# chaitjo/efficient-gnns

Hardware: NVIDIA H100
Metric: edges aggregated/s (fwd+bwd), 3-layer GCN student + logit-KD, ARXIV-shape (higher is better)
Workload: dtype f32

## Files before the change

### efficient-gnns_b200/csrc/gemm_tf32x3.cu

```cuda
#include <cuda.h>

#include "common.cuh"
#include "tc_common.cuh"

namespace b200gnn {
namespace gemm {
using namespace tc;

constexpr int BM = 128, BK = 32;
constexpr int THREADS = 384;
constexpr int CONSUMER_WARPS = 8;
constexpr int TILE_BYTES = BM * BK * 4;
constexpr int WG_TILE_BYTES = TILE_BYTES / 2;
constexpr int BAR_BYTES = 256;
constexpr int EPI_BYTES = CONSUMER_WARPS * 16 * 32 * 4;
constexpr int STAT_MAX_N = 256;
constexpr int STAT_BYTES = CONSUMER_WARPS * 2 * STAT_MAX_N * 4;
constexpr int XY_ROWS = 16;
constexpr int XY_SLOT_BYTES = 2 * XY_ROWS * 32 * 4;
constexpr int XY_BYTES = CONSUMER_WARPS * 2 * XY_SLOT_BYTES;
constexpr int XY_BAR_OFF = 128;
constexpr int BNBWD_TMA_MAX_K = 128;

template <int BN_T, int NSTAGE, int EXTRA = 0>
struct Cfg {
  static constexpr int BN = BN_T, STAGES = NSTAGE;
  static constexpr int B_TILE_BYTES = BN_T * BK * 4;
  static constexpr int STAGE_BYTES = 2 * TILE_BYTES + 2 * B_TILE_BYTES;
  static constexpr int ACC = BN_T / 2;
  static constexpr int SMEM_BYTES = NSTAGE * STAGE_BYTES + BAR_BYTES + EPI_BYTES + STAT_BYTES + EXTRA + 1024;
  static_assert(B_TILE_BYTES % 1024 == 0 && (BN_T == 128 || BN_T == 48), "tile shape (wgmma wrappers: N = 128, 48)");
  static_assert(2 * NSTAGE * 8 <= XY_BAR_OFF, "barrier block");
  static_assert(SMEM_BYTES <= 232448, "shared memory");
};

__device__ __forceinline__ void mma(float (&d)[64], uint64_t a, uint64_t b, uint32_t s) { wgmma_tf32_n128(d, a, b, s); }
__device__ __forceinline__ void mma(float (&d)[24], uint64_t a, uint64_t b, uint32_t s) { wgmma_tf32_n48(d, a, b, s); }

__device__ __forceinline__ int stg(int r, int c4) { return r * 32 + ((c4 ^ (r & 7)) << 2); }

struct Params {
  float* C;
  const float* bias;
  int64_t ldc;
  int32_t M, N, K;
  int32_t accumulate;
  float* Cp[16];
  int32_t n_peer, kc;
  int64_t row_off;
  int32_t bcast;
  int32_t stat_mode;
  float* stat_partial;
  const float* bn_x;
  const float* bn_y;
  const float* bn_mean;
  const float* bn_invstd;
  float inv_keep;
};

__device__ __forceinline__ void load_bn_chunk(const Params& p, int m0, int col, int q, int lane, float4 (&x)[4], float4 (&y)[4]) {
  if (col + 32 > p.N) return;
  const int sub = lane >> 3, cq = (lane & 7) * 4;
#pragma unroll
  for (int it = 0; it < 4; ++it) {
    const int grow = m0 + q * 16 + it * 4 + sub;
    if (grow < p.M) {
      const size_t o = (size_t)grow * p.ldc + col + cq;
      x[it] = __ldg(reinterpret_cast<const float4*>(p.bn_x + o));
      y[it] = __ldg(reinterpret_cast<const float4*>(p.bn_y + o));
    }
// ... 13 lines not shown
  uint64_t* bars = reinterpret_cast<uint64_t*>(smem + STAGES * STAGE_BYTES);
  uint64_t* full = bars;
  uint64_t* empty = bars + STAGES;
  float* epi_smem = reinterpret_cast<float*>(smem + STAGES * STAGE_BYTES + BAR_BYTES);
  float* stat_smem = reinterpret_cast<float*>(smem + STAGES * STAGE_BYTES + BAR_BYTES + EPI_BYTES);
  uint8_t* xy_smem = smem + STAGES * STAGE_BYTES + BAR_BYTES + EPI_BYTES + STAT_BYTES;
  uint64_t* xy_full = reinterpret_cast<uint64_t*>(smem + STAGES * STAGE_BYTES + XY_BAR_OFF);

  const int warp = threadIdx.x >> 5, lane = threadIdx.x & 31;

  if (threadIdx.x == 0) {
    for (int s = 0; s < STAGES; ++s) { mbar_init(&full[s], 1); mbar_init(&empty[s], 256); }
    if (XYTMA)
      for (int i = 0; i < 2 * CONSUMER_WARPS; ++i) mbar_init(&xy_full[i], 1);
    asm volatile("fence.mbarrier_init.release.cluster;" ::: "memory");
  }
  __syncthreads();

  const int num_m = (p.M + BM - 1) / BM, num_n = (p.N + BN - 1) / BN;
  const int num_tiles = num_m * num_n;
  const int num_kb = (p.K + BK - 1) / BK;

  if (warp < 4) {
    regs_dec<40>();
    if (threadIdx.x == 0) {
      int s = 0; uint32_t ph = 0;
      for (int tile = blockIdx.x; tile < num_tiles; tile += gridDim.x) {
        const int m0 = (tile / num_n) * BM, n0 = (tile % num_n) * BN;
        for (int kb = 0; kb < num_kb; ++kb) {
          mbar_wait(&empty[s], ph ^ 1);
          uint8_t* st = smem + s * STAGE_BYTES;
          mbar_expect_tx(&full[s], TILE_BYTES + 2 * B_TILE_BYTES);
          tma_load_2d(&tmA, &full[s], st, kb * BK, m0);
          tma_load_2d(&tmBhi, &full[s], st + 2 * TILE_BYTES, kb * BK, n0);
          tma_load_2d(&tmBlo, &full[s], st + 2 * TILE_BYTES + B_TILE_BYTES, kb * BK, n0);
          if (++s == STAGES) { s = 0; ph ^= 1; }
        }
      }
    }
    return;
  }
  regs_inc<232>();

  const int cw = (warp >> 2) - 1;
  const int t = threadIdx.x & 127;
  const int q = warp - 4;
  const bool vec_ok = PEER ? true : ((p.ldc % 4 == 0) && ((reinterpret_cast<uintptr_t>(p.C) & 15) == 0));
  float* stat = stat_smem + q * (2 * STAT_MAX_N);
  if (STAT) {
    for (int i = lane; i < 2 * p.N; i += 32) stat[i] = 0.f;
    __syncwarp();
  }
  constexpr int NCHUNK = (BN + 31) / 32;
  uint8_t* xy = xy_smem + q * (2 * XY_SLOT_BYTES);
  uint64_t* xyb = xy_full + q * 2;
  int n_mine = 0;
  if (XYTMA) {
    for (int tt = blockIdx.x; tt < num_tiles; tt += gridDim.x) n_mine += NCHUNK;
    if (lane == 0)
      for (int g = 0; g < 2 && g < n_mine; ++g) {
        const int tt = blockIdx.x + (g / NCHUNK) * gridDim.x, cc = g % NCHUNK;
        mbar_expect_tx(&xyb[g], XY_SLOT_BYTES);
        tma_load_2d(&tmX, &xyb[g], xy + g * XY_SLOT_BYTES, (tt % num_n) * BN + cc * 32, (tt / num_n) * BM + q * XY_ROWS);
        tma_load_2d(&tmY, &xyb[g], xy + g * XY_SLOT_BYTES + XY_SLOT_BYTES / 2, (tt % num_n) * BN + cc * 32,
                    (tt / num_n) * BM + q * XY_ROWS);
      }
  }
  float acc[ACC], sum[ACC];
  int s = 0; uint32_t ph = 0;
  int g_chunk = 0;
  for (int tile = blockIdx.x; tile < num_tiles; tile += gridDim.x) {
    const int m0 = (tile / num_n) * BM, n0 = (tile % num_n) * BN;
#pragma unroll
    for (int i = 0; i < ACC; ++i) sum[i] = 0.f;
    int prev = 0;
    for (int kb = 0; kb < num_kb; ++kb) {
      mbar_wait(&full[s], ph);
      uint8_t* st = smem + s * STAGE_BYTES;
      {
        uint4* hi = reinterpret_cast<uint4*>(st + cw * WG_TILE_BYTES);
        uint4* lo = reinterpret_cast<uint4*>(st + TILE_BYTES + cw * WG_TILE_BYTES);
#pragma unroll
        for (int i = 0; i < WG_TILE_BYTES / 16 / 128; ++i) {
          const int o = i * 128 + t;
          const uint4 v = hi[o];
          uint4 h, l;
          split4(v, h, l);
          hi[o] = h;
          lo[o] = l;
        }
      }
      asm volatile("fence.proxy.async.shared::cta;" ::: "memory");
      named_sync(1 + cw, 128);
      if (kb > 0) {
        wgmma_wait<0>();
        acc_fence(acc);
#pragma unroll
        for (int i = 0; i < ACC; ++i) sum[i] += acc[i];
        mbar_arrive(&empty[prev]);
      }
      wgmma_fence();
      const uint32_t sa = smem_u32(st);
#pragma unroll
      for (int k = 0; k < BK / 8; ++k) {
        const uint32_t koff = k * 32;
        const uint64_t a_hi = make_desc_k128(sa + cw * WG_TILE_BYTES + koff);
        const uint64_t a_lo = make_desc_k128(sa + TILE_BYTES + cw * WG_TILE_BYTES + koff);
        const uint64_t b_hi = make_desc_k128(sa + 2 * TILE_BYTES + koff);
        const uint64_t b_lo = make_desc_k128(sa + 2 * TILE_BYTES + B_TILE_BYTES + koff);
        mma(acc, a_lo, b_hi, k != 0);
        mma(acc, a_hi, b_lo, 1);
      }
#pragma unroll
      for (int k = 0; k < BK / 8; ++k) {
        const uint32_t koff = k * 32;
        mma(acc, make_desc_k128(sa + cw * WG_TILE_BYTES + koff), make_desc_k128(sa + 2 * TILE_BYTES + koff), 1);
      }
      wgmma_commit();
      prev = s;
      if (++s == STAGES) { s = 0; ph ^= 1; }
    }
    wgmma_wait<0>();
    acc_fence(acc);
#pragma unroll
    for (int i = 0; i < ACC; ++i) sum[i] += acc[i];
    mbar_arrive(&empty[prev]);

    float* tile_s = epi_smem + q * (16 * 32);
#pragma unroll
    for (int c = 0; c < NCHUNK; ++c, ++g_chunk) {
      const int col0 = n0 + c * 32;
      float4 xr[4], yr[4];
      if (STAT == 2) load_bn_chunk(p, m0, col0, q, lane, xr, yr);
#pragma unroll
      for (int jj = 0; jj < 4; ++jj) {
        const int j = c * 4 + jj;
        if (j * 8 < BN) {
          const int r0 = lane >> 2, cc = jj * 8 + 2 * (lane & 3);
          *reinterpret_cast<float2*>(tile_s + stg(r0, cc >> 2) + (cc & 3)) = make_float2(sum[4 * j], sum[4 * j + 1]);
          *reinterpret_cast<float2*>(tile_s + stg(r0 + 8, cc >> 2) + (cc & 3)) = make_float2(sum[4 * j + 2], sum[4 * j + 3]);
        }
      }
      __syncwarp();
      if (vec_ok && col0 + 32 <= p.N) {
        const float* xs = reinterpret_cast<const float*>(xy + (g_chunk & 1) * XY_SLOT_BYTES);
        const float* ys = xs + XY_ROWS * 32;
        if (XYTMA) mbar_wait(&xyb[g_chunk & 1], (uint32_t)((g_chunk >> 1) & 1));
        const int sub = lane >> 3, cq = (lane & 7) * 4;
        float4 b4 = make_float4(0.f, 0.f, 0.f, 0.f);
        if (p.bias) b4 = make_float4(__ldg(p.bias + col0 + cq), __ldg(p.bias + col0 + cq + 1), __ldg(p.bias + col0 + cq + 2),
                                     __ldg(p.bias + col0 + cq + 3));
        float4 s4 = make_float4(0.f, 0.f, 0.f, 0.f), q4 = s4, mu4 = s4, is4 = s4;
        if (BNB) {
// ... 136 lines not shown
}
}

using namespace b200gnn;

extern "C" int b200gnn_split_tf32_f32(const float* W, int64_t rows, int64_t cols, int transpose, float* hi, float* lo,
                                      void* stream) {
  if (!W || !hi || !lo || rows <= 0 || cols <= 0) return B200GNN_ERR_BAD_ARG;
  const int64_t n = rows * cols;
  int grid = (int)((n + 255) / 256);
  if (grid > 132 * 8) grid = 132 * 8;
  gemm::split_tf32_kernel<<<grid, 256, 0, (cudaStream_t)stream>>>(W, rows, cols, transpose, hi, lo);
  return check_launch();
}

static int g_bnbwd_variant = 0;
extern "C" void b200gnn_gemm_set_bnbwd_variant(int v) { g_bnbwd_variant = v; }

static int gemm_dispatch(const float* A, int64_t lda, const float* B_hi, const float* B_lo, int64_t ldb, float* C, int64_t ldc,
                         int64_t M, int64_t N, int64_t K, const float* bias, int accumulate, void* stream,
                         const gemm::Params* st = nullptr) {
  if (!A || !B_hi || !B_lo || !C || M <= 0 || N <= 0 || K <= 0 || lda < K || ldb < K || ldc < N ||
      M >= INT32_MAX || N >= INT32_MAX || K >= INT32_MAX)
    return B200GNN_ERR_BAD_ARG;
  if (lda % 4 || ldb % 4 || !aligned_to(A, 16) || !aligned_to(B_hi, 16) || !aligned_to(B_lo, 16))
    return B200GNN_ERR_UNSUPPORTED;
  gemm::Params p{};
  p.C = C; p.bias = bias; p.ldc = ldc; p.M = (int32_t)M; p.N = (int32_t)N; p.K = (int32_t)K; p.accumulate = accumulate ? 1 : 0;
  p.n_peer = 0; p.kc = 0; p.row_off = 0; p.bcast = 0;
  if (st) {
    if (N % 32 || N > gemm::STAT_MAX_N || N <= 48 || ldc % 4 || !aligned_to(C, 16) || !st->stat_partial) return B200GNN_ERR_UNSUPPORTED;
    p.stat_mode = st->stat_mode; p.stat_partial = st->stat_partial; p.bn_x = st->bn_x; p.bn_y = st->bn_y;
    p.bn_mean = st->bn_mean; p.bn_invstd = st->bn_invstd; p.inv_keep = st->inv_keep;
    if (p.stat_mode == 1) return gemm::launch<gemm::Cfg<128, 3>, 1>(A, lda, B_hi, B_lo, ldb, p, (cudaStream_t)stream);
    if (N % 128 == 0 && (g_bnbwd_variant == 1 || (g_bnbwd_variant == 0 && K < gemm::BNBWD_TMA_MAX_K)))
      return gemm::launch<gemm::Cfg<128, 2, gemm::XY_BYTES>, 3>(A, lda, B_hi, B_lo, ldb, p, (cudaStream_t)stream);
    return gemm::launch<gemm::Cfg<128, 3>, 2>(A, lda, B_hi, B_lo, ldb, p, (cudaStream_t)stream);
  }
  if (N <= 48) return gemm::launch<gemm::Cfg<48, 4>>(A, lda, B_hi, B_lo, ldb, p, (cudaStream_t)stream);
  return gemm::launch<gemm::Cfg<128, 3>>(A, lda, B_hi, B_lo, ldb, p, (cudaStream_t)stream);
}

extern "C" int64_t b200gnn_gemm_stat_slots(int64_t M, int64_t N) {
  if (M <= 0 || N <= 0) return B200GNN_ERR_BAD_ARG;
  int dev = 0, sms = 132;
  cudaGetDevice(&dev);
  cudaDeviceGetAttribute(&sms, cudaDevAttrMultiProcessorCount, dev);
  const int64_t tiles = ((M + gemm::BM - 1) / gemm::BM) * ((N + 127) / 128);
  return gemm::CONSUMER_WARPS * (tiles < sms ? tiles : sms);
}

extern "C" int b200gnn_gemm_tf32x3_stats_f32(const float* A, int64_t lda, const float* B_hi, const float* B_lo, int64_t ldb,
                                             float* C, int64_t ldc, int64_t M, int64_t N, int64_t K, const float* bias,
                                             int accumulate, float* partial, int64_t slots, void* stream) {
  if (!partial || slots < b200gnn_gemm_stat_slots(M, N) || (accumulate && bias)) return B200GNN_ERR_BAD_ARG;
  gemm::Params st{};
  st.stat_mode = 1; st.stat_partial = partial;
  return gemm_dispatch(A, lda, B_hi, B_lo, ldb, C, ldc, M, N, K, bias, accumulate, stream, &st);
}

extern "C" int b200gnn_gemm_tf32x3_bnbwd_f32(const float* A, int64_t lda, const float* B_hi, const float* B_lo, int64_t ldb,
                                             float* C, int64_t ldc, int64_t M, int64_t N, int64_t K, int accumulate,
                                             const float* Xout, const float* Y, const float* mean, const float* invstd, float p_drop,
                                             float* partial, int64_t slots, void* stream) {
  if (!partial || !Xout || !Y || !mean || !invstd || p_drop < 0.f || p_drop >= 1.f || slots < b200gnn_gemm_stat_slots(M, N))
    return B200GNN_ERR_BAD_ARG;
  if (!aligned_to(Xout, 16) || !aligned_to(Y, 16) || !aligned_to(mean, 16) || !aligned_to(invstd, 16)) return B200GNN_ERR_UNSUPPORTED;
  gemm::Params st{};
  st.stat_mode = 2; st.stat_partial = partial; st.bn_x = Xout; st.bn_y = Y; st.bn_mean = mean; st.bn_invstd = invstd;
  st.inv_keep = p_drop > 0.f ? 1.f / (1.f - p_drop) : 1.f;
  return gemm_dispatch(A, lda, B_hi, B_lo, ldb, C, ldc, M, N, K, nullptr, accumulate, stream, &st);
}

extern "C" int b200gnn_gemm_tf32x3_f32(const float* A, int64_t lda, const float* B_hi, const float* B_lo, int64_t ldb,
                                       float* C, int64_t ldc, int64_t M, int64_t N, int64_t K, const float* bias,
                                       void* stream) {
  return gemm_dispatch(A, lda, B_hi, B_lo, ldb, C, ldc, M, N, K, bias, 0, stream);
}

extern "C" int b200gnn_gemm_tf32x3_acc_f32(const float* A, int64_t lda, const float* B_hi, const float* B_lo, int64_t ldb,
                                           float* C, int64_t ldc, int64_t M, int64_t N, int64_t K, void* stream) {
  return gemm_dispatch(A, lda, B_hi, B_lo, ldb, C, ldc, M, N, K, nullptr, 1, stream);
}

extern "C" int b200gnn_gemm_tf32x3_scatter_f32(const float* A, int64_t lda, const float* B_hi, const float* B_lo, int64_t ldb,
                                               float* const* C_ptrs, int32_t world, int64_t row_off, int64_t M, int64_t N, int64_t K,
                                               const float* bias, void* stream) {
  if (!A || !B_hi || !B_lo || !C_ptrs || world <= 0 || world > 16 || M <= 0 || N <= 0 || K <= 0 || lda < K || ldb < K || row_off < 0 ||
      M >= INT32_MAX || N >= INT32_MAX || K >= INT32_MAX)
    return B200GNN_ERR_BAD_ARG;
  if (N % world || (N / world) % 32 || N <= 48) return B200GNN_ERR_UNSUPPORTED;
  if (lda % 4 || ldb % 4 || !aligned_to(A, 16) || !aligned_to(B_hi, 16) || !aligned_to(B_lo, 16)) return B200GNN_ERR_UNSUPPORTED;
  gemm::Params p{};
  p.C = nullptr; p.bias = bias; p.ldc = N; p.M = (int32_t)M; p.N = (int32_t)N; p.K = (int32_t)K; p.accumulate = 0;
  p.n_peer = world; p.kc = (int32_t)(N / world); p.row_off = row_off; p.bcast = 0;
  for (int q = 0; q < world; ++q) {
    if (!C_ptrs[q] || !aligned_to(C_ptrs[q], 16)) return B200GNN_ERR_BAD_ARG;
    p.Cp[q] = C_ptrs[q];
  }
  return gemm::launch<gemm::Cfg<128, 3>, 0, true>(A, lda, B_hi, B_lo, ldb, p, (cudaStream_t)stream);
}

extern "C" int b200gnn_gemm_tf32x3_bcast_f32(const float* A, int64_t lda, const float* B_hi, const float* B_lo, int64_t ldb,
                                             float* const* C_ptrs, int32_t world, int64_t row_off, int64_t ldc, int64_t M, int64_t N,
                                             int64_t K, const float* bias, void* stream) {
  if (!A || !B_hi || !B_lo || !C_ptrs || world <= 0 || world > 16 || M <= 0 || N <= 0 || K <= 0 || lda < K || ldb < K || ldc < N ||
      row_off < 0 || M >= INT32_MAX || N >= INT32_MAX || K >= INT32_MAX)
    return B200GNN_ERR_BAD_ARG;
  if (lda % 4 || ldb % 4 || ldc % 4 || !aligned_to(A, 16) || !aligned_to(B_hi, 16) || !aligned_to(B_lo, 16)) return B200GNN_ERR_UNSUPPORTED;
  gemm::Params p{};
  p.C = C_ptrs[0]; p.bias = bias; p.ldc = ldc; p.M = (int32_t)M; p.N = (int32_t)N; p.K = (int32_t)K; p.accumulate = 0;
  p.n_peer = world; p.kc = (int32_t)N; p.row_off = row_off; p.bcast = 1;
  for (int q = 0; q < world; ++q) {
    if (!C_ptrs[q] || !aligned_to(C_ptrs[q], 16)) return B200GNN_ERR_BAD_ARG;
    p.Cp[q] = C_ptrs[q];
  }
  if (N <= 48) return gemm::launch<gemm::Cfg<48, 4>, 0, true>(A, lda, B_hi, B_lo, ldb, p, (cudaStream_t)stream);
  return gemm::launch<gemm::Cfg<128, 3>, 0, true>(A, lda, B_hi, B_lo, ldb, p, (cudaStream_t)stream);
}
```

### efficient-gnns_b200/csrc/gemm_wgrad_tf32x3.cu

```cuda
#include "common.cuh"
#include "tc_common.cuh"

namespace b200gnn {
namespace wgrad {
using namespace tc;

constexpr int BKN = 32;
constexpr int TM = 128, TN = 128;
constexpr int THREADS = 384;
constexpr int STAGES = 3;
constexpr int RAW_BYTES = BKN * (TM + TN) * 4;
constexpr int OP_BYTES = 128 * BKN * 4;
constexpr int T_BYTES = 4 * OP_BYTES;
constexpr int SMEM_BYTES = STAGES * RAW_BYTES + 2 * T_BYTES + 256 + 1024;
constexpr int MAX_RANGES = 132;
constexpr int64_t MAX_PARTIAL_FLOATS = (int64_t)MAX_RANGES * 256 * 256;
constexpr int MAX_KIN = 2048, MAX_NOUT = 512;
static_assert(SMEM_BYTES <= 232448, "shared memory");

struct Params {
  float* partial;
  int32_t Nn, Kin, Kpad, Nout, Npad, num_kb;
  int32_t n_tn, n_ranges;
};

__global__ void __launch_bounds__(THREADS, 1)
wgrad_tf32x3_kernel(const __grid_constant__ CUtensorMap tmX, const __grid_constant__ CUtensorMap tmG, const Params p) {
  extern __shared__ uint8_t smem_raw[];
  uint8_t* smem = reinterpret_cast<uint8_t*>((reinterpret_cast<uintptr_t>(smem_raw) + 1023) & ~(uintptr_t)1023);
  uint8_t* tbuf = smem + STAGES * RAW_BYTES;
  uint64_t* full = reinterpret_cast<uint64_t*>(tbuf + 2 * T_BYTES);
  uint64_t* empty = full + STAGES;

  const int tiles = (p.Kpad / TM) * p.n_tn;
  const int tile = (int)blockIdx.x % tiles, range = (int)blockIdx.x / tiles;
  const int mt = tile / p.n_tn, nt = tile % p.n_tn;
  const int kb0 = (int)((int64_t)p.num_kb * range / p.n_ranges);
  const int kb1 = (int)((int64_t)p.num_kb * (range + 1) / p.n_ranges);

  const int warp = threadIdx.x >> 5, lane = threadIdx.x & 31;
  if (threadIdx.x == 0) {
    for (int s = 0; s < STAGES; ++s) { mbar_init(&full[s], 1); mbar_init(&empty[s], 256); }
    asm volatile("fence.mbarrier_init.release.cluster;" ::: "memory");
  }
  __syncthreads();

  if (warp < 4) {
    regs_dec<40>();
    if (threadIdx.x == 0) {
      int s = 0; uint32_t ph = 0;
      for (int kb = kb0; kb < kb1; ++kb) {
        mbar_wait(&empty[s], ph ^ 1);
        uint8_t* st = smem + s * RAW_BYTES;
        mbar_expect_tx(&full[s], RAW_BYTES);
        tma_load_2d(&tmX, &full[s], st, mt * TM, kb * BKN);
        tma_load_2d(&tmG, &full[s], st + BKN * TM * 4, nt * TN, kb * BKN);
        if (++s == STAGES) { s = 0; ph ^= 1; }
      }
    }
    return;
  }
  regs_inc<232>();

  const int cw = (warp >> 2) - 1;
  const int ct = threadIdx.x - 128;
  float acc[64], sum[64];
#pragma unroll
  for (int i = 0; i < 64; ++i) sum[i] = 0.f;
  int s = 0; uint32_t ph = 0;
  for (int kb = kb0, i = 0; kb < kb1; ++kb, ++i) {
    mbar_wait(&full[s], ph);
    const float* rx = reinterpret_cast<const float*>(smem + s * RAW_BYTES);
    const float* rg = rx + BKN * TM;
    uint8_t* T = tbuf + (i & 1) * T_BYTES;
#pragma unroll
    for (int u = 0; u < 8; ++u) {
      const int idx = u * 256 + ct;
      const int op = idx >> 10, r = idx & 127, c = (idx >> 7) & 7;
      const float* src = (op ? rg : rx) + (4 * c) * 128 + r;
      const uint4 v = make_uint4(__float_as_uint(src[0]), __float_as_uint(src[128]), __float_as_uint(src[256]),
                                 __float_as_uint(src[384]));
      uint4 h, l;
      split4(v, h, l);
      uint8_t* base = T + op * 2 * OP_BYTES;
      *reinterpret_cast<uint4*>(base + swz128(r, c)) = h;
      *reinterpret_cast<uint4*>(base + OP_BYTES + swz128(r, c)) = l;
    }
    asm volatile("fence.proxy.async.shared::cta;" ::: "memory");
    mbar_arrive(&empty[s]);
    if (i > 0) {
      wgmma_wait<0>();
      acc_fence(acc);
#pragma unroll
      for (int j = 0; j < 64; ++j) sum[j] += acc[j];
    }
    named_sync(1, 256);
    wgmma_fence();
    const uint32_t sa = smem_u32(T);
#pragma unroll
    for (int k = 0; k < BKN / 8; ++k) {
      const uint32_t koff = k * 32;
      const uint64_t x_hi = make_desc_k128(sa + cw * (OP_BYTES / 2) + koff);
      const uint64_t x_lo = make_desc_k128(sa + OP_BYTES + cw * (OP_BYTES / 2) + koff);
      const uint64_t g_hi = make_desc_k128(sa + 2 * OP_BYTES + koff);
      const uint64_t g_lo = make_desc_k128(sa + 3 * OP_BYTES + koff);
      wgmma_tf32_n128(acc, x_lo, g_hi, k != 0);
      wgmma_tf32_n128(acc, x_hi, g_lo, 1);
    }
#pragma unroll
    for (int k = 0; k < BKN / 8; ++k) {
      const uint32_t koff = k * 32;
      wgmma_tf32_n128(acc, make_desc_k128(sa + cw * (OP_BYTES / 2) + koff), make_desc_k128(sa + 2 * OP_BYTES + koff), 1);
    }
    wgmma_commit();
    if (++s == STAGES) { s = 0; ph ^= 1; }
  }
  if (kb1 > kb0) {
    wgmma_wait<0>();
    acc_fence(acc);
#pragma unroll
    for (int j = 0; j < 64; ++j) sum[j] += acc[j];
  }
  float* out = p.partial + (size_t)range * p.Kpad * p.Npad;
  const int row0 = mt * TM + cw * 64 + (warp & 3) * 16 + (lane >> 2);
#pragma unroll
  for (int j = 0; j < 16; ++j) {
    const int col = nt * TN + 8 * j + 2 * (lane & 3);
    if (col < p.Npad) {
      *reinterpret_cast<float2*>(out + (size_t)row0 * p.Npad + col) = make_float2(sum[4 * j], sum[4 * j + 1]);
      *reinterpret_cast<float2*>(out + (size_t)(row0 + 8) * p.Npad + col) = make_float2(sum[4 * j + 2], sum[4 * j + 3]);
    }
  }
}

constexpr int RED_VECS = 32, RED_GROUPS = 8;
__global__ void __launch_bounds__(RED_VECS * RED_GROUPS) wgrad_reduce_kernel(const float4* __restrict__ partial, int n_part,
                                                                             int Kin, int Kpad, int Nout, int Npad,
                                                                             float* __restrict__ out) {
  __shared__ float4 sh[RED_GROUPS][RED_VECS];
  const int64_t n_vec = (int64_t)Kpad * Npad / 4;
  const int v = threadIdx.x % RED_VECS, g = threadIdx.x / RED_VECS;
  const int64_t i = (int64_t)blockIdx.x * RED_VECS + v;
  float4 acc = make_float4(0.f, 0.f, 0.f, 0.f);
  if (i < n_vec)
    for (int c = g; c < n_part; c += RED_GROUPS) {
      const float4 x = __ldcs(partial + (size_t)c * n_vec + i);
      acc.x += x.x; acc.y += x.y; acc.z += x.z; acc.w += x.w;
    }
  sh[g][v] = acc;
  __syncthreads();
  if (g != 0 || i >= n_vec) return;
  const int row = (int)(i / (Npad / 4)), c4 = (int)(i % (Npad / 4)) * 4;
  if (c4 >= Nout || row >= Kin) return;
#pragma unroll
  for (int j = 1; j < RED_GROUPS; ++j) {
    const float4 x = sh[j][v];
    acc.x += x.x; acc.y += x.y; acc.z += x.z; acc.w += x.w;
  }
  *reinterpret_cast<float4*>(out + (size_t)row * Nout + c4) = acc;
}

static bool make_map_rows(CUtensorMap* m, const float* base, int64_t rows, int64_t width, int64_t ld) {
  EncodeTiledFn fn = encode_fn();
  if (!fn) return false;
  cuuint64_t dims[2] = {(cuuint64_t)width, (cuuint64_t)rows};
  cuuint64_t strides[1] = {(cuuint64_t)ld * 4};
  cuuint32_t box[2] = {128, (cuuint32_t)BKN};
  cuuint32_t estr[2] = {1, 1};
  return fn(m, CU_TENSOR_MAP_DATA_TYPE_FLOAT32, 2, const_cast<float*>(base), dims, strides, box, estr,
            CU_TENSOR_MAP_INTERLEAVE_NONE, CU_TENSOR_MAP_SWIZZLE_NONE, CU_TENSOR_MAP_L2_PROMOTION_L2_256B,
            CU_TENSOR_MAP_FLOAT_OOB_FILL_NONE) == CUDA_SUCCESS;
}

static int64_t pad_k(int64_t Kin) { return (Kin + TM - 1) / TM * TM; }
static int64_t pad_n(int64_t Nout) { return (Nout + 31) / 32 * 32; }
static int range_cap(int64_t Kin, int64_t Nout) {
  const int64_t c = MAX_PARTIAL_FLOATS / (pad_k(Kin) * pad_n(Nout));
  return (int)(c > MAX_RANGES ? MAX_RANGES : (c < 1 ? 1 : c));
}

}
}

using namespace b200gnn;

extern "C" int64_t b200gnn_wgrad_workspace_floats(int64_t Kin, int64_t Nout) {
  if (Kin <= 0 || Nout <= 0) return B200GNN_ERR_BAD_ARG;
  if (Kin > wgrad::MAX_KIN || Nout > wgrad::MAX_NOUT) return B200GNN_ERR_UNSUPPORTED;
  return wgrad::range_cap(Kin, Nout) * wgrad::pad_k(Kin) * wgrad::pad_n(Nout);
}

extern "C" int b200gnn_gemm_wgrad_tf32x3_f32(const float* X, int64_t ldx, const float* G, int64_t ldg, float* dW,
                                             int64_t Nn, int64_t Kin, int64_t Nout, float* workspace, void* stream) {
  if (!X || !G || !dW || !workspace || Nn <= 0 || Kin <= 0 || Nout <= 0 || ldx < Kin || ldg < Nout || Nn >= INT32_MAX)
    return B200GNN_ERR_BAD_ARG;
  if (Kin % 4 || Kin > wgrad::MAX_KIN || Nout % 4 || Nout > wgrad::MAX_NOUT || ldx % 4 || ldg % 4 || !aligned_to(X, 16) || !aligned_to(G, 16) ||
      !aligned_to(dW, 16) || !aligned_to(workspace, 16))
    return B200GNN_ERR_UNSUPPORTED;
  CUtensorMap tX, tG;
  if (!wgrad::make_map_rows(&tX, X, Nn, Kin, ldx) || !wgrad::make_map_rows(&tG, G, Nn, Nout, ldg)) return B200GNN_ERR_UNSUPPORTED;
  int dev = 0, sms = 132;
  cudaGetDevice(&dev);
  static bool attr_set[64] = {};
  if (dev >= 0 && dev < 64 && !attr_set[dev]) {
    cudaError_t e = cudaFuncSetAttribute(wgrad::wgrad_tf32x3_kernel, cudaFuncAttributeMaxDynamicSharedMemorySize,
                                         wgrad::SMEM_BYTES);
    if (e != cudaSuccess) { set_cuda_error(e); return B200GNN_ERR_CUDA; }
    attr_set[dev] = true;
  }
  cudaDeviceGetAttribute(&sms, cudaDevAttrMultiProcessorCount, dev);
  cudaStream_t st = (cudaStream_t)stream;
  wgrad::Params p;
  p.partial = workspace; p.Nn = (int32_t)Nn; p.Kin = (int32_t)Kin; p.Nout = (int32_t)Nout;
  p.Kpad = (int32_t)wgrad::pad_k(Kin);
  p.Npad = (int32_t)wgrad::pad_n(Nout);
  p.num_kb = (int32_t)((Nn + wgrad::BKN - 1) / wgrad::BKN);
  p.n_tn = (p.Npad + wgrad::TN - 1) / wgrad::TN;
  const int tiles = (int)(p.Kpad / wgrad::TM) * p.n_tn;
  int ranges = sms / tiles;
  const int cap = wgrad::range_cap(Kin, Nout);
  if (ranges > cap) ranges = cap;
  if (ranges > p.num_kb) ranges = p.num_kb;
  if (ranges < 1) ranges = 1;
  p.n_ranges = ranges;
  int rc;
  wgrad::wgrad_tf32x3_kernel<<<tiles * ranges, wgrad::THREADS, wgrad::SMEM_BYTES, st>>>(tX, tG, p);
  if ((rc = check_launch())) return rc;
  const int64_t n_vec = (int64_t)p.Kpad * p.Npad / 4;
  wgrad::wgrad_reduce_kernel<<<(int)((n_vec + wgrad::RED_VECS - 1) / wgrad::RED_VECS), wgrad::RED_VECS * wgrad::RED_GROUPS, 0, st>>>(
      reinterpret_cast<const float4*>(workspace), ranges, (int)Kin, p.Kpad, (int)Nout, p.Npad, dW);
  return check_launch();
}
```

### efficient-gnns_b200/csrc/tc_common.cuh

```cuda
#pragma once
#include <cuda.h>
#include <cuda_runtime.h>
#include <stdint.h>

namespace b200gnn {
namespace tc {

constexpr uint32_t TF32_MASK = 0xFFFFE000u;

__device__ __forceinline__ uint32_t smem_u32(const void* p) { return (uint32_t)__cvta_generic_to_shared(p); }

__device__ __forceinline__ void mbar_init(uint64_t* bar, uint32_t count) {
  asm volatile("mbarrier.init.shared::cta.b64 [%0], %1;" ::"r"(smem_u32(bar)), "r"(count));
}
__device__ __forceinline__ void mbar_arrive(uint64_t* bar) {
  asm volatile("mbarrier.arrive.shared::cta.b64 _, [%0];" ::"r"(smem_u32(bar)) : "memory");
}
__device__ __forceinline__ void mbar_expect_tx(uint64_t* bar, uint32_t bytes) {
  asm volatile("mbarrier.arrive.expect_tx.shared::cta.b64 _, [%0], %1;" ::"r"(smem_u32(bar)), "r"(bytes) : "memory");
}
__device__ __forceinline__ bool mbar_try_wait(uint64_t* bar, uint32_t parity) {
  uint32_t ok;
  asm volatile(
      "{\n\t"
      ".reg .pred p;\n\t"
      "mbarrier.try_wait.parity.shared::cta.b64 p, [%1], %2;\n\t"
      "selp.u32 %0, 1, 0, p;\n\t"
      "}"
      : "=r"(ok)
      : "r"(smem_u32(bar)), "r"(parity)
      : "memory");
  return ok != 0;
}
__device__ __forceinline__ void mbar_wait(uint64_t* bar, uint32_t parity) {
  while (!mbar_try_wait(bar, parity)) {}
}

__device__ __forceinline__ void tma_load_2d(const CUtensorMap* tmap, uint64_t* bar, void* dst, int c0, int c1) {
  asm volatile(
      "cp.async.bulk.tensor.2d.shared::cluster.global.mbarrier::complete_tx::bytes [%0], [%1, {%3, %4}], [%2];"
      ::"r"(smem_u32(dst)), "l"(reinterpret_cast<uint64_t>(tmap)), "r"(smem_u32(bar)), "r"(c0), "r"(c1)
      : "memory");
}

__device__ __forceinline__ void named_sync(uint32_t id, uint32_t count) {
  asm volatile("bar.sync %0, %1;" ::"r"(id), "r"(count) : "memory");
}

template <uint32_t N> __device__ __forceinline__ void regs_dec() { asm volatile("setmaxnreg.dec.sync.aligned.u32 %0;" ::"n"(N)); }
template <uint32_t N> __device__ __forceinline__ void regs_inc() { asm volatile("setmaxnreg.inc.sync.aligned.u32 %0;" ::"n"(N)); }

__device__ __forceinline__ uint64_t make_desc_k128(uint32_t saddr) {
  uint64_t d = 0;
  d |= (uint64_t)((saddr & 0x3FFFF) >> 4);
  d |= (uint64_t)1 << 16;
  d |= (uint64_t)(1024 >> 4) << 32;
  d |= (uint64_t)1 << 62;
  return d;
}
__device__ __forceinline__ uint32_t swz128(int r, int c) { return (uint32_t)(r * 128 + ((c ^ (r & 7)) << 4)); }

__device__ __forceinline__ void wgmma_fence() { asm volatile("wgmma.fence.sync.aligned;" ::: "memory"); }
__device__ __forceinline__ void wgmma_commit() { asm volatile("wgmma.commit_group.sync.aligned;" ::: "memory"); }
template <int N> __device__ __forceinline__ void wgmma_wait() { asm volatile("wgmma.wait_group.sync.aligned %0;" ::"n"(N) : "memory"); }
template <int R> __device__ __forceinline__ void acc_fence(float (&d)[R]) {
#pragma unroll
  for (int i = 0; i < R; ++i) asm volatile("" : "+f"(d[i])::"memory");
}

__device__ __forceinline__ void wgmma_tf32_n128(float (&d)[64], uint64_t da, uint64_t db, uint32_t scale_d) {
  asm volatile(
      "{\n\t.reg .pred p;\n\tsetp.ne.b32 p, %66, 0;\n\t"
      "wgmma.mma_async.sync.aligned.m64n128k8.f32.tf32.tf32 {%0,%1,%2,%3,%4,%5,%6,%7,%8,%9,%10,%11,%12,%13,%14,%15,%16,%17,%18,%19,%20,%21,%22,%23,%24,%25,%26,%27,%28,%29,%30,%31,%32,%33,%34,%35,%36,%37,%38,%39,%40,%41,%42,%43,%44,%45,%46,%47,%48,%49,%50,%51,%52,%53,%54,%55,%56,%57,%58,%59,%60,%61,%62,%63}, %64, %65, p, 1, 1;\n\t}"
      : "+f"(d[0]), "+f"(d[1]), "+f"(d[2]), "+f"(d[3]), "+f"(d[4]), "+f"(d[5]), "+f"(d[6]), "+f"(d[7]), "+f"(d[8]), "+f"(d[9]), "+f"(d[10]), "+f"(d[11]), "+f"(d[12]), "+f"(d[13]), "+f"(d[14]), "+f"(d[15]), "+f"(d[16]), "+f"(d[17]), "+f"(d[18]), "+f"(d[19]), "+f"(d[20]), "+f"(d[21]), "+f"(d[22]), "+f"(d[23]), "+f"(d[24]), "+f"(d[25]), "+f"(d[26]), "+f"(d[27]), "+f"(d[28]), "+f"(d[29]), "+f"(d[30]), "+f"(d[31]), "+f"(d[32]), "+f"(d[33]), "+f"(d[34]), "+f"(d[35]), "+f"(d[36]), "+f"(d[37]), "+f"(d[38]), "+f"(d[39]), "+f"(d[40]), "+f"(d[41]), "+f"(d[42]), "+f"(d[43]), "+f"(d[44]), "+f"(d[45]), "+f"(d[46]), "+f"(d[47]), "+f"(d[48]), "+f"(d[49]), "+f"(d[50]), "+f"(d[51]), "+f"(d[52]), "+f"(d[53]), "+f"(d[54]), "+f"(d[55]), "+f"(d[56]), "+f"(d[57]), "+f"(d[58]), "+f"(d[59]), "+f"(d[60]), "+f"(d[61]), "+f"(d[62]), "+f"(d[63])
      : "l"(da), "l"(db), "r"(scale_d));
}
__device__ __forceinline__ void wgmma_tf32_n48(float (&d)[24], uint64_t da, uint64_t db, uint32_t scale_d) {
  asm volatile(
      "{\n\t.reg .pred p;\n\tsetp.ne.b32 p, %26, 0;\n\t"
      "wgmma.mma_async.sync.aligned.m64n48k8.f32.tf32.tf32 {%0,%1,%2,%3,%4,%5,%6,%7,%8,%9,%10,%11,%12,%13,%14,%15,%16,%17,%18,%19,%20,%21,%22,%23}, %24, %25, p, 1, 1;\n\t}"
      : "+f"(d[0]), "+f"(d[1]), "+f"(d[2]), "+f"(d[3]), "+f"(d[4]), "+f"(d[5]), "+f"(d[6]), "+f"(d[7]), "+f"(d[8]), "+f"(d[9]), "+f"(d[10]), "+f"(d[11]), "+f"(d[12]), "+f"(d[13]), "+f"(d[14]), "+f"(d[15]), "+f"(d[16]), "+f"(d[17]), "+f"(d[18]), "+f"(d[19]), "+f"(d[20]), "+f"(d[21]), "+f"(d[22]), "+f"(d[23])
      : "l"(da), "l"(db), "r"(scale_d));
}

__device__ __forceinline__ uint32_t rna_tf32(float x) { return (__float_as_uint(x) + 0x1000u) & TF32_MASK; }
__device__ __forceinline__ void split1(uint32_t v, uint32_t& h, uint32_t& l) {
  h = rna_tf32(__uint_as_float(v));
  l = rna_tf32(__uint_as_float(v) - __uint_as_float(h));
}
__device__ __forceinline__ void split4(const uint4& v, uint4& h, uint4& l) {
  split1(v.x, h.x, l.x); split1(v.y, h.y, l.y); split1(v.z, h.z, l.z); split1(v.w, h.w, l.w);
}

typedef CUresult (*EncodeTiledFn)(CUtensorMap*, CUtensorMapDataType, cuuint32_t, void*, const cuuint64_t*, const cuuint64_t*,
                                  const cuuint32_t*, const cuuint32_t*, CUtensorMapInterleave, CUtensorMapSwizzle,
                                  CUtensorMapL2promotion, CUtensorMapFloatOOBfill);

inline EncodeTiledFn encode_fn() {
  static EncodeTiledFn fn = nullptr;
  if (!fn) {
    void* p = nullptr;
    cudaDriverEntryPointQueryResult q;
    if (cudaGetDriverEntryPoint("cuTensorMapEncodeTiled", &p, cudaEnableDefault, &q) == cudaSuccess &&
        q == cudaDriverEntryPointSuccess)
      fn = reinterpret_cast<EncodeTiledFn>(p);
  }
  return fn;
}

}
}
```

Before: 3.063 billion.

## Feed A operand to wgmma from registers and split hi/lo in registers

Switches both the forward GEMM and the weight-gradient GEMM to register-sourced wgmma for the A operand. Each thread loads its A fragment from shared memory and splits it into TF32 hi/lo parts in registers, instead of writing the split back into shared memory and fencing. Double-buffered register fragments, alternating between stages, keep in-flight wgmma operands intact. The smaller per-stage footprint allows deeper pipelines (3→4, 4→6, 3→5 stages), at the cost of more registers and many 32-bit shared loads, some of them possibly bank-conflicted.

```diff
diff --git a/efficient-gnns_b200/csrc/gemm_tf32x3.cu b/efficient-gnns_b200/csrc/gemm_tf32x3.cu
--- a/efficient-gnns_b200/csrc/gemm_tf32x3.cu
+++ b/efficient-gnns_b200/csrc/gemm_tf32x3.cu
@@ -11,7 +11,6 @@
 constexpr int THREADS = 384;
 constexpr int CONSUMER_WARPS = 8;
 constexpr int TILE_BYTES = BM * BK * 4;
-constexpr int WG_TILE_BYTES = TILE_BYTES / 2;
 constexpr int BAR_BYTES = 256;
 constexpr int EPI_BYTES = CONSUMER_WARPS * 16 * 32 * 4;
 constexpr int STAT_MAX_N = 256;
@@ -26,7 +25,7 @@
 struct Cfg {
   static constexpr int BN = BN_T, STAGES = NSTAGE;
   static constexpr int B_TILE_BYTES = BN_T * BK * 4;
-  static constexpr int STAGE_BYTES = 2 * TILE_BYTES + 2 * B_TILE_BYTES;
+  static constexpr int STAGE_BYTES = TILE_BYTES + 2 * B_TILE_BYTES;
   static constexpr int ACC = BN_T / 2;
   static constexpr int SMEM_BYTES = NSTAGE * STAGE_BYTES + BAR_BYTES + EPI_BYTES + STAT_BYTES + EXTRA + 1024;
   static_assert(B_TILE_BYTES % 1024 == 0 && (BN_T == 128 || BN_T == 48), "tile shape (wgmma wrappers: N = 128, 48)");
@@ -34,8 +33,17 @@
   static_assert(SMEM_BYTES <= 232448, "shared memory");
 };
 
-__device__ __forceinline__ void mma(float (&d)[64], uint64_t a, uint64_t b, uint32_t s) { wgmma_tf32_n128(d, a, b, s); }
-__device__ __forceinline__ void mma(float (&d)[24], uint64_t a, uint64_t b, uint32_t s) { wgmma_tf32_n48(d, a, b, s); }
+__device__ __forceinline__ void mma(float (&d)[64], const uint32_t (&a)[4], uint64_t b, uint32_t s) { wgmma_tf32_n128_rs(d, a, b, s); }
+__device__ __forceinline__ void mma(float (&d)[24], const uint32_t (&a)[4], uint64_t b, uint32_t s) { wgmma_tf32_n48_rs(d, a, b, s); }
+
+__device__ __forceinline__ uint32_t a_frag_offset(int r0, int lane) { return r0 * 128 + ((lane >> 2) << 4) + (lane & 3) * 4; }
+__device__ __forceinline__ void load_a(uint32_t frag, uint32_t (&v)[BK / 8][4]) {
+  asm("" : "+r"(frag));
+#pragma unroll
+  for (int k = 0; k < BK / 8; ++k)
+#pragma unroll
+    for (int i = 0; i < 4; ++i) v[k][i] = lds32((frag ^ ((2 * k + (i >> 1)) << 4)) + (i & 1) * 8 * 128);
+}
 
 __device__ __forceinline__ int stg(int r, int c4) { return r * 32 + ((c4 ^ (r & 7)) << 2); }
 
@@ -115,8 +123,8 @@
           uint8_t* st = smem + s * STAGE_BYTES;
           mbar_expect_tx(&full[s], TILE_BYTES + 2 * B_TILE_BYTES);
           tma_load_2d(&tmA, &full[s], st, kb * BK, m0);
-          tma_load_2d(&tmBhi, &full[s], st + 2 * TILE_BYTES, kb * BK, n0);
-          tma_load_2d(&tmBlo, &full[s], st + 2 * TILE_BYTES + B_TILE_BYTES, kb * BK, n0);
+          tma_load_2d(&tmBhi, &full[s], st + TILE_BYTES, kb * BK, n0);
+          tma_load_2d(&tmBlo, &full[s], st + TILE_BYTES + B_TILE_BYTES, kb * BK, n0);
           if (++s == STAGES) { s = 0; ph ^= 1; }
         }
       }
@@ -125,8 +133,6 @@
   }
   regs_inc<232>();
 
-  const int cw = (warp >> 2) - 1;
-  const int t = threadIdx.x & 127;
   const int q = warp - 4;
   const bool vec_ok = PEER ? true : ((p.ldc % 4 == 0) && ((reinterpret_cast<uintptr_t>(p.C) & 15) == 0));
   float* stat = stat_smem + q * (2 * STAT_MAX_N);
@@ -150,31 +156,24 @@
       }
   }
   float acc[ACC], sum[ACC];
+  uint32_t ah0[BK / 8][4], al0[BK / 8][4], ah1[BK / 8][4], al1[BK / 8][4];
+  const uint32_t frag = a_frag_offset(q * 16 + (lane >> 2), lane);
   int s = 0; uint32_t ph = 0;
   int g_chunk = 0;
   for (int tile = blockIdx.x; tile < num_tiles; tile += gridDim.x) {
     const int m0 = (tile / num_n) * BM, n0 = (tile % num_n) * BN;
 #pragma unroll
-    for (int i = 0; i < ACC; ++i) sum[i] = 0.f;
+    for (int i = 0; i < ACC; ++i) sum[i] = acc[i] = 0.f;
     int prev = 0;
-    for (int kb = 0; kb < num_kb; ++kb) {
+    auto stage = [&](int kb, uint32_t (&h)[BK / 8][4], uint32_t (&l)[BK / 8][4]) {
       mbar_wait(&full[s], ph);
       uint8_t* st = smem + s * STAGE_BYTES;
-      {
-        uint4* hi = reinterpret_cast<uint4*>(st + cw * WG_TILE_BYTES);
-        uint4* lo = reinterpret_cast<uint4*>(st + TILE_BYTES + cw * WG_TILE_BYTES);
-#pragma unroll
-        for (int i = 0; i < WG_TILE_BYTES / 16 / 128; ++i) {
-          const int o = i * 128 + t;
-          const uint4 v = hi[o];
-          uint4 h, l;
-          split4(v, h, l);
-          hi[o] = h;
-          lo[o] = l;
-        }
-      }
-      asm volatile("fence.proxy.async.shared::cta;" ::: "memory");
-      named_sync(1 + cw, 128);
+      load_a(smem_u32(st) + frag, h);
+#pragma unroll
+      for (int k = 0; k < BK / 8; ++k)
+#pragma unroll
+        for (int i = 0; i < 4; ++i) split1(h[k][i], h[k][i], l[k][i]);
+      reg_fence(h); reg_fence(l);
       if (kb > 0) {
         wgmma_wait<0>();
         acc_fence(acc);
@@ -183,25 +182,22 @@
         mbar_arrive(&empty[prev]);
       }
       wgmma_fence();
-      const uint32_t sa = smem_u32(st);
+      const uint32_t sb = smem_u32(st + TILE_BYTES);
 #pragma unroll
       for (int k = 0; k < BK / 8; ++k) {
         const uint32_t koff = k * 32;
-        const uint64_t a_hi = make_desc_k128(sa + cw * WG_TILE_BYTES + koff);
-        const uint64_t a_lo = make_desc_k128(sa + TILE_BYTES + cw * WG_TILE_BYTES + koff);
-        const uint64_t b_hi = make_desc_k128(sa + 2 * TILE_BYTES + koff);
-        const uint64_t b_lo = make_desc_k128(sa + 2 * TILE_BYTES + B_TILE_BYTES + koff);
-        mma(acc, a_lo, b_hi, k != 0);
-        mma(acc, a_hi, b_lo, 1);
-      }
-#pragma unroll
-      for (int k = 0; k < BK / 8; ++k) {
-        const uint32_t koff = k * 32;
-        mma(acc, make_desc_k128(sa + cw * WG_TILE_BYTES + koff), make_desc_k128(sa + 2 * TILE_BYTES + koff), 1);
-      }
+        mma(acc, l[k], make_desc_k128(sb + koff), k != 0);
+        mma(acc, h[k], make_desc_k128(sb + B_TILE_BYTES + koff), 1);
+      }
+#pragma unroll
+      for (int k = 0; k < BK / 8; ++k) mma(acc, h[k], make_desc_k128(sb + k * 32), 1);
       wgmma_commit();
       prev = s;
       if (++s == STAGES) { s = 0; ph ^= 1; }
+    };
+    for (int kb = 0; kb < num_kb; kb += 2) {
+      stage(kb, ah0, al0);
+      if (kb + 1 < num_kb) stage(kb + 1, ah1, al1);
     }
     wgmma_wait<0>();
     acc_fence(acc);
@@ -404,13 +400,13 @@
     if (N % 32 || N > gemm::STAT_MAX_N || N <= 48 || ldc % 4 || !aligned_to(C, 16) || !st->stat_partial) return B200GNN_ERR_UNSUPPORTED;
     p.stat_mode = st->stat_mode; p.stat_partial = st->stat_partial; p.bn_x = st->bn_x; p.bn_y = st->bn_y;
     p.bn_mean = st->bn_mean; p.bn_invstd = st->bn_invstd; p.inv_keep = st->inv_keep;
-    if (p.stat_mode == 1) return gemm::launch<gemm::Cfg<128, 3>, 1>(A, lda, B_hi, B_lo, ldb, p, (cudaStream_t)stream);
+    if (p.stat_mode == 1) return gemm::launch<gemm::Cfg<128, 4>, 1>(A, lda, B_hi, B_lo, ldb, p, (cudaStream_t)stream);
     if (N % 128 == 0 && (g_bnbwd_variant == 1 || (g_bnbwd_variant == 0 && K < gemm::BNBWD_TMA_MAX_K)))
       return gemm::launch<gemm::Cfg<128, 2, gemm::XY_BYTES>, 3>(A, lda, B_hi, B_lo, ldb, p, (cudaStream_t)stream);
-    return gemm::launch<gemm::Cfg<128, 3>, 2>(A, lda, B_hi, B_lo, ldb, p, (cudaStream_t)stream);
-  }
-  if (N <= 48) return gemm::launch<gemm::Cfg<48, 4>>(A, lda, B_hi, B_lo, ldb, p, (cudaStream_t)stream);
-  return gemm::launch<gemm::Cfg<128, 3>>(A, lda, B_hi, B_lo, ldb, p, (cudaStream_t)stream);
+    return gemm::launch<gemm::Cfg<128, 4>, 2>(A, lda, B_hi, B_lo, ldb, p, (cudaStream_t)stream);
+  }
+  if (N <= 48) return gemm::launch<gemm::Cfg<48, 6>>(A, lda, B_hi, B_lo, ldb, p, (cudaStream_t)stream);
+  return gemm::launch<gemm::Cfg<128, 4>>(A, lda, B_hi, B_lo, ldb, p, (cudaStream_t)stream);
 }
 
 extern "C" int64_t b200gnn_gemm_stat_slots(int64_t M, int64_t N) {
@@ -470,7 +466,7 @@
     if (!C_ptrs[q] || !aligned_to(C_ptrs[q], 16)) return B200GNN_ERR_BAD_ARG;
     p.Cp[q] = C_ptrs[q];
   }
-  return gemm::launch<gemm::Cfg<128, 3>, 0, true>(A, lda, B_hi, B_lo, ldb, p, (cudaStream_t)stream);
+  return gemm::launch<gemm::Cfg<128, 4>, 0, true>(A, lda, B_hi, B_lo, ldb, p, (cudaStream_t)stream);
 }
 
 extern "C" int b200gnn_gemm_tf32x3_bcast_f32(const float* A, int64_t lda, const float* B_hi, const float* B_lo, int64_t ldb,
@@ -487,6 +483,6 @@
     if (!C_ptrs[q] || !aligned_to(C_ptrs[q], 16)) return B200GNN_ERR_BAD_ARG;
     p.Cp[q] = C_ptrs[q];
   }
-  if (N <= 48) return gemm::launch<gemm::Cfg<48, 4>, 0, true>(A, lda, B_hi, B_lo, ldb, p, (cudaStream_t)stream);
-  return gemm::launch<gemm::Cfg<128, 3>, 0, true>(A, lda, B_hi, B_lo, ldb, p, (cudaStream_t)stream);
-}
+  if (N <= 48) return gemm::launch<gemm::Cfg<48, 6>, 0, true>(A, lda, B_hi, B_lo, ldb, p, (cudaStream_t)stream);
+  return gemm::launch<gemm::Cfg<128, 4>, 0, true>(A, lda, B_hi, B_lo, ldb, p, (cudaStream_t)stream);
+}
diff --git a/efficient-gnns_b200/csrc/gemm_wgrad_tf32x3.cu b/efficient-gnns_b200/csrc/gemm_wgrad_tf32x3.cu
--- a/efficient-gnns_b200/csrc/gemm_wgrad_tf32x3.cu
+++ b/efficient-gnns_b200/csrc/gemm_wgrad_tf32x3.cu
@@ -8,10 +8,11 @@
 constexpr int BKN = 32;
 constexpr int TM = 128, TN = 128;
 constexpr int THREADS = 384;
-constexpr int STAGES = 3;
+constexpr int STAGES = 5;
+constexpr int X_BOX = 8;
 constexpr int RAW_BYTES = BKN * (TM + TN) * 4;
 constexpr int OP_BYTES = 128 * BKN * 4;
-constexpr int T_BYTES = 4 * OP_BYTES;
+constexpr int T_BYTES = 2 * OP_BYTES;
 constexpr int SMEM_BYTES = STAGES * RAW_BYTES + 2 * T_BYTES + 256 + 1024;
 constexpr int MAX_RANGES = 132;
 constexpr int64_t MAX_PARTIAL_FLOATS = (int64_t)MAX_RANGES * 256 * 256;
@@ -53,7 +54,8 @@
         mbar_wait(&empty[s], ph ^ 1);
         uint8_t* st = smem + s * RAW_BYTES;
         mbar_expect_tx(&full[s], RAW_BYTES);
-        tma_load_2d(&tmX, &full[s], st, mt * TM, kb * BKN);
+        for (int j = 0; j < TM / X_BOX; ++j)
+          tma_load_2d(&tmX, &full[s], st + j * BKN * X_BOX * 4, mt * TM + j * X_BOX, kb * BKN);
         tma_load_2d(&tmG, &full[s], st + BKN * TM * 4, nt * TN, kb * BKN);
         if (++s == STAGES) { s = 0; ph ^= 1; }
       }
@@ -64,28 +66,34 @@
 
   const int cw = (warp >> 2) - 1;
   const int ct = threadIdx.x - 128;
+  const uint32_t xfrag = (8 * cw + 2 * (warp & 3)) * (BKN * X_BOX * 4) + (lane & 3) * (X_BOX * 4) + (lane >> 2) * 4;
   float acc[64], sum[64];
 #pragma unroll
-  for (int i = 0; i < 64; ++i) sum[i] = 0.f;
+  for (int i = 0; i < 64; ++i) sum[i] = acc[i] = 0.f;
+  uint32_t xh0[BKN / 8][4], xl0[BKN / 8][4], xh1[BKN / 8][4], xl1[BKN / 8][4];
   int s = 0; uint32_t ph = 0;
-  for (int kb = kb0, i = 0; kb < kb1; ++kb, ++i) {
+  auto block = [&](int i, uint32_t (&h)[BKN / 8][4], uint32_t (&l)[BKN / 8][4]) {
     mbar_wait(&full[s], ph);
-    const float* rx = reinterpret_cast<const float*>(smem + s * RAW_BYTES);
-    const float* rg = rx + BKN * TM;
+    const uint32_t sraw = smem_u32(smem + s * RAW_BYTES);
+    const float* rg = reinterpret_cast<const float*>(smem + s * RAW_BYTES + BKN * TM * 4);
     uint8_t* T = tbuf + (i & 1) * T_BYTES;
 #pragma unroll
-    for (int u = 0; u < 8; ++u) {
+    for (int u = 0; u < 4; ++u) {
       const int idx = u * 256 + ct;
-      const int op = idx >> 10, r = idx & 127, c = (idx >> 7) & 7;
-      const float* src = (op ? rg : rx) + (4 * c) * 128 + r;
+      const int r = idx & 127, c = idx >> 7;
+      const float* src = rg + (4 * c) * 128 + r;
       const uint4 v = make_uint4(__float_as_uint(src[0]), __float_as_uint(src[128]), __float_as_uint(src[256]),
                                  __float_as_uint(src[384]));
-      uint4 h, l;
-      split4(v, h, l);
-      uint8_t* base = T + op * 2 * OP_BYTES;
-      *reinterpret_cast<uint4*>(base + swz128(r, c)) = h;
-      *reinterpret_cast<uint4*>(base + OP_BYTES + swz128(r, c)) = l;
-    }
+      uint4 hv, lv;
+      split4(v, hv, lv);
+      *reinterpret_cast<uint4*>(T + swz128(r, c)) = hv;
+      *reinterpret_cast<uint4*>(T + OP_BYTES + swz128(r, c)) = lv;
+    }
+#pragma unroll
+    for (int k = 0; k < BKN / 8; ++k)
+#pragma unroll
+      for (int j = 0; j < 4; ++j)
+        split1(lds32(sraw + xfrag + (j & 1) * (BKN * X_BOX * 4) + (8 * k + 4 * (j >> 1)) * (X_BOX * 4)), h[k][j], l[k][j]);
     asm volatile("fence.proxy.async.shared::cta;" ::: "memory");
     mbar_arrive(&empty[s]);
     if (i > 0) {
@@ -95,25 +103,23 @@
       for (int j = 0; j < 64; ++j) sum[j] += acc[j];
     }
     named_sync(1, 256);
+    reg_fence(h); reg_fence(l);
     wgmma_fence();
     const uint32_t sa = smem_u32(T);
 #pragma unroll
     for (int k = 0; k < BKN / 8; ++k) {
       const uint32_t koff = k * 32;
-      const uint64_t x_hi = make_desc_k128(sa + cw * (OP_BYTES / 2) + koff);
-      const uint64_t x_lo = make_desc_k128(sa + OP_BYTES + cw * (OP_BYTES / 2) + koff);
-      const uint64_t g_hi = make_desc_k128(sa + 2 * OP_BYTES + koff);
-      const uint64_t g_lo = make_desc_k128(sa + 3 * OP_BYTES + koff);
-      wgmma_tf32_n128(acc, x_lo, g_hi, k != 0);
-      wgmma_tf32_n128(acc, x_hi, g_lo, 1);
-    }
-#pragma unroll
-    for (int k = 0; k < BKN / 8; ++k) {
-      const uint32_t koff = k * 32;
-      wgmma_tf32_n128(acc, make_desc_k128(sa + cw * (OP_BYTES / 2) + koff), make_desc_k128(sa + 2 * OP_BYTES + koff), 1);
-    }
+      wgmma_tf32_n128_rs(acc, l[k], make_desc_k128(sa + koff), k != 0);
+      wgmma_tf32_n128_rs(acc, h[k], make_desc_k128(sa + OP_BYTES + koff), 1);
+    }
+#pragma unroll
+    for (int k = 0; k < BKN / 8; ++k) wgmma_tf32_n128_rs(acc, h[k], make_desc_k128(sa + k * 32), 1);
     wgmma_commit();
     if (++s == STAGES) { s = 0; ph ^= 1; }
+  };
+  for (int i = 0; i < kb1 - kb0; i += 2) {
+    block(i, xh0, xl0);
+    if (i + 1 < kb1 - kb0) block(i + 1, xh1, xl1);
   }
   if (kb1 > kb0) {
     wgmma_wait<0>();
@@ -160,12 +166,12 @@
   *reinterpret_cast<float4*>(out + (size_t)row * Nout + c4) = acc;
 }
 
-static bool make_map_rows(CUtensorMap* m, const float* base, int64_t rows, int64_t width, int64_t ld) {
+static bool make_map_rows(CUtensorMap* m, const float* base, int64_t rows, int64_t width, int64_t ld, int box_cols) {
   EncodeTiledFn fn = encode_fn();
   if (!fn) return false;
   cuuint64_t dims[2] = {(cuuint64_t)width, (cuuint64_t)rows};
   cuuint64_t strides[1] = {(cuuint64_t)ld * 4};
-  cuuint32_t box[2] = {128, (cuuint32_t)BKN};
+  cuuint32_t box[2] = {(cuuint32_t)box_cols, (cuuint32_t)BKN};
   cuuint32_t estr[2] = {1, 1};
   return fn(m, CU_TENSOR_MAP_DATA_TYPE_FLOAT32, 2, const_cast<float*>(base), dims, strides, box, estr,
             CU_TENSOR_MAP_INTERLEAVE_NONE, CU_TENSOR_MAP_SWIZZLE_NONE, CU_TENSOR_MAP_L2_PROMOTION_L2_256B,
@@ -198,7 +204,8 @@
       !aligned_to(dW, 16) || !aligned_to(workspace, 16))
     return B200GNN_ERR_UNSUPPORTED;
   CUtensorMap tX, tG;
-  if (!wgrad::make_map_rows(&tX, X, Nn, Kin, ldx) || !wgrad::make_map_rows(&tG, G, Nn, Nout, ldg)) return B200GNN_ERR_UNSUPPORTED;
+  if (!wgrad::make_map_rows(&tX, X, Nn, Kin, ldx, wgrad::X_BOX) || !wgrad::make_map_rows(&tG, G, Nn, Nout, ldg, wgrad::TN))
+    return B200GNN_ERR_UNSUPPORTED;
   int dev = 0, sms = 132;
   cudaGetDevice(&dev);
   static bool attr_set[64] = {};
diff --git a/efficient-gnns_b200/csrc/tc_common.cuh b/efficient-gnns_b200/csrc/tc_common.cuh
--- a/efficient-gnns_b200/csrc/tc_common.cuh
+++ b/efficient-gnns_b200/csrc/tc_common.cuh
@@ -43,6 +43,12 @@
       : "memory");
 }
 
+__device__ __forceinline__ uint32_t lds32(uint32_t saddr) {
+  uint32_t v;
+  asm volatile("ld.shared.b32 %0, [%1];" : "=r"(v) : "r"(saddr) : "memory");
+  return v;
+}
+
 __device__ __forceinline__ void named_sync(uint32_t id, uint32_t count) {
   asm volatile("bar.sync %0, %1;" ::"r"(id), "r"(count) : "memory");
 }
@@ -68,19 +74,25 @@
   for (int i = 0; i < R; ++i) asm volatile("" : "+f"(d[i])::"memory");
 }
 
-__device__ __forceinline__ void wgmma_tf32_n128(float (&d)[64], uint64_t da, uint64_t db, uint32_t scale_d) {
+__device__ __forceinline__ void wgmma_tf32_n128_rs(float (&d)[64], const uint32_t (&a)[4], uint64_t db, uint32_t scale_d) {
   asm volatile(
-      "{\n\t.reg .pred p;\n\tsetp.ne.b32 p, %66, 0;\n\t"
-      "wgmma.mma_async.sync.aligned.m64n128k8.f32.tf32.tf32 {%0,%1,%2,%3,%4,%5,%6,%7,%8,%9,%10,%11,%12,%13,%14,%15,%16,%17,%18,%19,%20,%21,%22,%23,%24,%25,%26,%27,%28,%29,%30,%31,%32,%33,%34,%35,%36,%37,%38,%39,%40,%41,%42,%43,%44,%45,%46,%47,%48,%49,%50,%51,%52,%53,%54,%55,%56,%57,%58,%59,%60,%61,%62,%63}, %64, %65, p, 1, 1;\n\t}"
+      "{\n\t.reg .pred p;\n\tsetp.ne.b32 p, %69, 0;\n\t"
+      "wgmma.mma_async.sync.aligned.m64n128k8.f32.tf32.tf32 {%0,%1,%2,%3,%4,%5,%6,%7,%8,%9,%10,%11,%12,%13,%14,%15,%16,%17,%18,%19,%20,%21,%22,%23,%24,%25,%26,%27,%28,%29,%30,%31,%32,%33,%34,%35,%36,%37,%38,%39,%40,%41,%42,%43,%44,%45,%46,%47,%48,%49,%50,%51,%52,%53,%54,%55,%56,%57,%58,%59,%60,%61,%62,%63}, {%64,%65,%66,%67}, %68, p, 1, 1;\n\t}"
       : "+f"(d[0]), "+f"(d[1]), "+f"(d[2]), "+f"(d[3]), "+f"(d[4]), "+f"(d[5]), "+f"(d[6]), "+f"(d[7]), "+f"(d[8]), "+f"(d[9]), "+f"(d[10]), "+f"(d[11]), "+f"(d[12]), "+f"(d[13]), "+f"(d[14]), "+f"(d[15]), "+f"(d[16]), "+f"(d[17]), "+f"(d[18]), "+f"(d[19]), "+f"(d[20]), "+f"(d[21]), "+f"(d[22]), "+f"(d[23]), "+f"(d[24]), "+f"(d[25]), "+f"(d[26]), "+f"(d[27]), "+f"(d[28]), "+f"(d[29]), "+f"(d[30]), "+f"(d[31]), "+f"(d[32]), "+f"(d[33]), "+f"(d[34]), "+f"(d[35]), "+f"(d[36]), "+f"(d[37]), "+f"(d[38]), "+f"(d[39]), "+f"(d[40]), "+f"(d[41]), "+f"(d[42]), "+f"(d[43]), "+f"(d[44]), "+f"(d[45]), "+f"(d[46]), "+f"(d[47]), "+f"(d[48]), "+f"(d[49]), "+f"(d[50]), "+f"(d[51]), "+f"(d[52]), "+f"(d[53]), "+f"(d[54]), "+f"(d[55]), "+f"(d[56]), "+f"(d[57]), "+f"(d[58]), "+f"(d[59]), "+f"(d[60]), "+f"(d[61]), "+f"(d[62]), "+f"(d[63])
-      : "l"(da), "l"(db), "r"(scale_d));
+      : "r"(a[0]), "r"(a[1]), "r"(a[2]), "r"(a[3]), "l"(db), "r"(scale_d));
 }
-__device__ __forceinline__ void wgmma_tf32_n48(float (&d)[24], uint64_t da, uint64_t db, uint32_t scale_d) {
+__device__ __forceinline__ void wgmma_tf32_n48_rs(float (&d)[24], const uint32_t (&a)[4], uint64_t db, uint32_t scale_d) {
   asm volatile(
-      "{\n\t.reg .pred p;\n\tsetp.ne.b32 p, %26, 0;\n\t"
-      "wgmma.mma_async.sync.aligned.m64n48k8.f32.tf32.tf32 {%0,%1,%2,%3,%4,%5,%6,%7,%8,%9,%10,%11,%12,%13,%14,%15,%16,%17,%18,%19,%20,%21,%22,%23}, %24, %25, p, 1, 1;\n\t}"
+      "{\n\t.reg .pred p;\n\tsetp.ne.b32 p, %29, 0;\n\t"
+      "wgmma.mma_async.sync.aligned.m64n48k8.f32.tf32.tf32 {%0,%1,%2,%3,%4,%5,%6,%7,%8,%9,%10,%11,%12,%13,%14,%15,%16,%17,%18,%19,%20,%21,%22,%23}, {%24,%25,%26,%27}, %28, p, 1, 1;\n\t}"
       : "+f"(d[0]), "+f"(d[1]), "+f"(d[2]), "+f"(d[3]), "+f"(d[4]), "+f"(d[5]), "+f"(d[6]), "+f"(d[7]), "+f"(d[8]), "+f"(d[9]), "+f"(d[10]), "+f"(d[11]), "+f"(d[12]), "+f"(d[13]), "+f"(d[14]), "+f"(d[15]), "+f"(d[16]), "+f"(d[17]), "+f"(d[18]), "+f"(d[19]), "+f"(d[20]), "+f"(d[21]), "+f"(d[22]), "+f"(d[23])
-      : "l"(da), "l"(db), "r"(scale_d));
+      : "r"(a[0]), "r"(a[1]), "r"(a[2]), "r"(a[3]), "l"(db), "r"(scale_d));
+}
+template <int K> __device__ __forceinline__ void reg_fence(uint32_t (&r)[K][4]) {
+#pragma unroll
+  for (int k = 0; k < K; ++k)
+#pragma unroll
+    for (int i = 0; i < 4; ++i) asm volatile("" : "+r"(r[k][i])::"memory");
 }
 
 __device__ __forceinline__ uint32_t rna_tf32(float x) { return (__float_as_uint(x) + 0x1000u) & TF32_MASK; }
```

Measured after the change: 3.189 billion (median of 6 runs). 1.04x the previous value.
